# NVlabs/intrinsic3d

Measured on NVIDIA H100. Metric: gauss_newton_iterations_per_sec, higher is better.
Workload: dtype f32

## Files before the change

intrinsic3d_b200/csrc/i3d_engine.cu:

```cuda
#include <cuda_runtime.h>
#include <dlfcn.h>

#include <algorithm>
#include <chrono>
#include <climits>
#include <cmath>
#include <cstdarg>
#include <cstdio>
#include <cstdlib>
#include <cstring>
#include <string>
#include <vector>

#include "../../include/i3d_c_api.h"
#include "i3d_kernels.cuh"
#include "i3d_lighting.cuh"
#include "i3d_recolor.cuh"
#include "i3d_gridops.cuh"
#include "i3d_host.h"
#include "i3d_frames.h"
#include "i3d_fusion.h"
#include "i3d_mesh.h"
#include "i3d_render.h"
#include "i3d_texture.h"
#include "i3d_distance.h"
#include "i3d_grid_from_mesh.h"
#include "i3d_raster.h"
#include "i3d_track.h"

using namespace i3d;

#define I3D_ABI_VERSION 1

namespace
{
std::string g_create_error;

struct NcclApi
{
    typedef struct { char internal[128]; } UniqueId;
    typedef void* Comm;
    int (*GetUniqueId)(UniqueId*) = nullptr;
    int (*CommInitRank)(Comm*, int, UniqueId, int) = nullptr;
    int (*CommDestroy)(Comm) = nullptr;
    int (*AllReduce)(const void*, void*, size_t, int, int, Comm, cudaStream_t) = nullptr;
    const char* (*GetErrorString)(int) = nullptr;
    void* handle = nullptr;
    bool load(std::string* err)
    {
        if (handle) return true;
        const char* names[] = {"libnccl.so.2", "libnccl.so"};
        for (const char* nm : names) { handle = dlopen(nm, RTLD_NOW | RTLD_GLOBAL); if (handle) break; }
        if (!handle) { *err = std::string("cannot dlopen libnccl.so.2: ") + dlerror(); return false; }
        GetUniqueId = reinterpret_cast<decltype(GetUniqueId)>(dlsym(handle, "ncclGetUniqueId"));
        CommInitRank = reinterpret_cast<decltype(CommInitRank)>(dlsym(handle, "ncclCommInitRank"));
        CommDestroy = reinterpret_cast<decltype(CommDestroy)>(dlsym(handle, "ncclCommDestroy"));
        AllReduce = reinterpret_cast<decltype(AllReduce)>(dlsym(handle, "ncclAllReduce"));
        GetErrorString = reinterpret_cast<decltype(GetErrorString)>(dlsym(handle, "ncclGetErrorString"));
        if (!GetUniqueId || !CommInitRank || !CommDestroy || !AllReduce || !GetErrorString) { *err = "libnccl.so.2 lacks required symbols"; return false; }
        return true;
    }
};
NcclApi g_nccl;
// ... 287 lines not shown
    rows.n_active = e->n_active; rows.K = e->K; rows.stride = e->stride; rows.act = e->act.p; rows.Jt = e->Jt.p; rows.Jtail = e->Jtail.p;
    rows.row_frame = e->row_frame.p; rows.row_res = e->row_res.p; rows.row_wraw = e->row_wraw.p;
    return rows;
}

RegView reg_view(I3DEngine* e, const I3DParams& P)
{
    RegView rv;
    rv.flags = e->flags.p; rv.ea_w = e->ea_w.p; rv.lap = e->lap.p;
    rv.use_er = P.use_er; rv.use_es = P.use_es; rv.use_ea = P.use_ea;
    return rv;
}

SelectCam select_cam(const I3DEngine* e, const double hc9[9], float occlusion)
{
    SelectCam sc;
    sc.fx = static_cast<float>(hc9[0] * e->pyr_scale); sc.fy = static_cast<float>(hc9[1] * e->pyr_scale);
    sc.cx = static_cast<float>(hc9[2] * e->pyr_scale); sc.cy = static_cast<float>(hc9[3] * e->pyr_scale);
    sc.dist_zero = 1;
    for (int k = 0; k < 5; ++k) { sc.d[k] = static_cast<float>(hc9[4 + k]); if (sc.d[k] != 0.0f) sc.dist_zero = 0; }
    sc.occlusion = occlusion;
    return sc;
}

CullView cull_view(const I3DEngine* e, unsigned long long* stats)
{
    static const bool no_cull = std::getenv("I3D_NO_CULL") != nullptr;
    return CullView{e->tile_min.p, e->tile_max.p, no_cull ? 0 : 1, stats};
}

#define NK(call)                                                            \
    do {                                                                    \
        int _r = (call);                                                    \
        if (_r != 0) throw NcclError{_r, __LINE__};                         \
    } while (0)


bool pdl_enabled() { static const bool on = [] { const char* v = std::getenv("I3D_PDL"); return !(v && v[0] == '0'); }(); return on; }

template <bool COOPERATIVE = false, class... KArgs, class... Args>
void pdl_launch(I3DEngine* e, void (*kern)(KArgs...), unsigned grid, unsigned block, size_t smem, Args&&... args)
{
    cudaLaunchConfig_t cfg{};
    cfg.gridDim = dim3(grid); cfg.blockDim = dim3(block); cfg.dynamicSmemBytes = smem; cfg.stream = e->stream;
    cudaLaunchAttribute at[2];
    unsigned na = 0;
    if (COOPERATIVE) { at[na].id = cudaLaunchAttributeCooperative; at[na].val.cooperative = 1; ++na; }
    if (pdl_enabled()) { at[na].id = cudaLaunchAttributeProgrammaticStreamSerialization; at[na].val.programmaticStreamSerializationAllowed = 1; ++na; }
    cfg.attrs = at; cfg.numAttrs = na;
    CK(cudaLaunchKernelEx(&cfg, kern, static_cast<KArgs>(args)...));
    e->launches += 1;
}

template <int MODE>
void launch_eg_rows(I3DEngine* e, const GridView& g, const CamView& cv, const EgRows& rows, const int32_t* obs_frame, const float* obs_w)
{
    if constexpr (MODE == ROWS_COST)
    {
        const size_t smem = rows_smem_bytes(MODE, 256, true, e->F);
        if (2 * (smem + 1024) <= 227u * 1024u)
        {
            auto kern = k_eg_rows<MODE, 256, true>;
            CK(cudaFuncSetAttribute(kern, cudaFuncAttributeMaxDynamicSharedMemorySize, static_cast<int>(smem)));
            pdl_launch(e, kern, blocks_for(static_cast<size_t>(rows.stride), 256), 256, smem, g, e->frame_view(), cv, rows, obs_frame, obs_w, e->site(SITE_EG_COST));
            return;
        }
    }
    auto kern = k_eg_rows<MODE, 128, false>;
    const size_t smem = rows_smem_bytes(MODE, 128, false, e->F);
    CK(cudaFuncSetAttribute(kern, cudaFuncAttributeMaxDynamicSharedMemorySize, static_cast<int>(smem)));
    pdl_launch(e, kern, blocks_for(static_cast<size_t>(rows.stride), 128), 128, smem, g, e->frame_view(), cv, rows, obs_frame, obs_w, e->site(SITE_EG_COST));
}

void allreduce_scalars(I3DEngine* e, double* dev, int count, int kind, int respect_done)
{
    if (e->world <= 1) return;
    if (e->p2p_ready && count <= 30)
    {
        const unsigned int seq = ++e->xseq;
        pdl_launch(e, k_xchg_scalars, 1, 32, 0, e->p2p_view(), seq, dev, count, e->ctl.p, kind, respect_done);
        return;
    }
    NK(g_nccl.AllReduce(dev, dev, static_cast<size_t>(count), NCCL_FLOAT64, NCCL_SUM, e->comm, e->stream));
    if (kind >= 0) pdl_launch(e, k_epilogue, 1, 32, 0, e->ctl.p, dev, kind, respect_done);
}

void exchange(I3DEngine* e, float* v0, float* v1, float* extra_f, int n_extra_f, double* extra_d, int n_extra_d, int respect_done, int epilogue_kind = -1)
{
    if (e->world <= 1) return;
    const ShareView shv = e->share_view();
    const size_t nv = v1 ? 2 : 1;
    const size_t total = nv * static_cast<size_t>(e->n_shared) + n_extra_f + n_extra_d;
    const size_t threads = static_cast<size_t>(e->n_shared) + n_extra_f + n_extra_d;
    if (e->p2p_ready && total <= e->mbox_cap)
    {
        const unsigned int seq = ++e->xseq;
        double* buf = reinterpret_cast<double*>(e->mbox.p + I3DEngine::kMboxFlagBytes) + static_cast<size_t>(seq & 1u) * e->mbox_cap;
        pdl_launch(e, k_pack, blocks_for(threads), kThreads, 0, shv, v0, v1, extra_f, n_extra_f, extra_d, n_extra_d, buf, e->ctl.p, respect_done);
        pdl_launch(e, k_xchg_pull, blocks_for(threads), kThreads, 0, e->p2p_view(), seq, shv, v0, v1, extra_f, n_extra_f, extra_d, n_extra_d, e->ctl.p, respect_done, epilogue_kind);
        return;
    }
    e->xbuf.ensure(2 * static_cast<size_t>(e->n_shared) + CamAccLayout{e->F}.size() + 64);
    pdl_launch(e, k_pack, blocks_for(threads), kThreads, 0, shv, v0, v1, extra_f, n_extra_f, extra_d, n_extra_d, e->xbuf.p, e->ctl.p, respect_done);
    NK(g_nccl.AllReduce(e->xbuf.p, e->xbuf.p, total, NCCL_FLOAT64, NCCL_SUM, e->comm, e->stream));
    pdl_launch(e, k_unpack, blocks_for(threads), kThreads, 0, shv, v0, v1, extra_f, n_extra_f, extra_d, n_extra_d, e->xbuf.p, e->ctl.p, respect_done);
    if (epilogue_kind >= 0) pdl_launch(e, k_epilogue, 1, 32, 0, e->ctl.p, extra_d, epilogue_kind, respect_done);
// ... 70 lines not shown
        if (smem > dyn_max) break;
        int occ0 = 0, occ1 = 0;
        CK(cudaOccupancyMaxActiveBlocksPerMultiprocessor(&occ0, k_cg_step<false>, kStepThreads, smem));
        CK(cudaOccupancyMaxActiveBlocksPerMultiprocessor(&occ1, k_cg_step<true>, kStepThreads, smem));
        if (std::min(occ0, occ1) < bps) continue;
        if (static_cast<size_t>(bps) * sms + 8 > e->max_blocks) break;
        e->step_grid = static_cast<unsigned>(bps * sms); e->step_K = static_cast<int>(K); e->step_smem = smem;
        return true;
    }
    return false;
}

template <bool INIT>
void launch_cg_step(I3DEngine* e, const GridView& g, const RegView& rv, const SolveVecs& sv, float dmin, float dmax)
{
    const int64_t items = (e->n + 3) / 4;
    pdl_launch<true>(e, k_cg_step<INIT>, e->step_grid, kStepThreads, e->step_smem, g, rv, sv, items, e->step_K, e->type_w.p, e->minv.p, dmin, dmax,
                     e->ctl.p, e->site(SITE_OP_POST), e->site(SITE_EG_APPLY).out, e->site(SITE_UPDATE));
}

int gn_iteration_impl(I3DEngine* e, const I3DParams& P, I3DIterInfo& info)
{
    std::memset(&info, 0, sizeof(info));
    if (e->n <= 0) return fail(e, "i3d_gn_iteration: no grid uploaded");
    if (e->F <= 0) return fail(e, "i3d_gn_iteration: no frames uploaded");
    if (!e->have_cam) return fail(e, "i3d_gn_iteration: camera not set");
    if (!e->have_sh) return fail(e, "i3d_gn_iteration: SH coefficients not set");
    if (e->world > 1 && !e->shard_ready) return fail(e, "i3d_gn_iteration: world > 1 but i3d_set_shard was not called after the grid/frames upload");
    int K = P.num_observations;
    if (K <= 0 || K > e->F) K = e->F;
    if (K > I3D_MAX_OBS) return fail(e, "i3d_gn_iteration: num_observations (%d) exceeds I3D_MAX_OBS (%d)", K, I3D_MAX_OBS);
    if (P.lm_steps < 1) return fail(e, "i3d_gn_iteration: lm_steps < 1");
    if (P.residual_reset_period < 1) return fail(e, "i3d_gn_iteration: residual_reset_period < 1");
    if (check_frame_limit(e, e->F, K) != 0) return 1;
    e->K = K;
    e->last_params = P;
    e->timing.phases.clear(); begin_timing(e->timing, {}); e->launches = 0; e->host_syncs = 0;
    const int64_t n = e->n;
    const int F = e->F;
    const bool multi = e->world > 1;
    cudaStream_t st = e->stream;
    ensure_vectors(e);
    e->iter_dev.ensure(1);
    const Shard sh = e->shard();
    const int64_t own = sh.own_end - sh.own_begin;
    const int64_t hc = e->held_count();
    const size_t U = static_cast<size_t>(e->U());
    Timer t_total(e->timing, e->stream, "total");
    auto sync = [&]() { CK(cudaStreamSynchronize(st)); e->host_syncs += 1; };

    Timer t_sel(e->timing, e->stream, "select");
    e->flags.ensure(n);
    GridView g = e->grid_view(e->sdf, e->alb);
    pdl_launch(e, k_flags, blocks_for(static_cast<size_t>(sh.loc_end - sh.loc_begin)), kThreads, 0, g, sh, P.thres_shell, P.fix_all_albedo, e->flags.p);
    const int nscan = std::max(1, static_cast<int>((own + kScanChunk - 1) / kScanChunk));
    e->scan_counts.ensure(nscan); e->scan_total.ensure(1); e->act.ensure(n);
    pdl_launch(e, k_scan_count, nscan, kThreads, 0, own, e->flags.p + sh.own_begin, FL_ROW, e->scan_counts.p);
    pdl_launch(e, k_scan_blocks, 1, 1024, 0, nscan, e->scan_counts.p, e->scan_total.p);
    pdl_launch(e, k_scan_scatter, nscan, kThreads, 0, own, e->flags.p + sh.own_begin, FL_ROW, e->scan_counts.p, e->act.p, static_cast<int32_t>(sh.own_begin));
    const CamAccLayout lay{F};
    CK(cudaMemsetAsync(e->v_bg.p, 0, U * sizeof(float), st));
    CK(cudaMemsetAsync(e->v_cg.p, 0, U * sizeof(float), st));
    CK(cudaMemsetAsync(e->v_qg.p, 0, U * sizeof(float), st));
    CK(cudaMemsetAsync(e->v_delta.p, 0, U * sizeof(float), st));
    CK(cudaMemsetAsync(e->v_tr.p, 0, static_cast<size_t>(n) * sizeof(float), st));
    CK(cudaMemsetAsync(e->cam_acc.p, 0, lay.size() * sizeof(float), st));
    CK(cudaMemsetAsync(e->v_bgd.p, 0, U * sizeof(double), st));
    CK(cudaMemsetAsync(e->v_cgd.p, 0, U * sizeof(double), st));
    CK(cudaMemsetAsync(e->v_qgd.p, 0, U * sizeof(double), st));
    CK(cudaMemsetAsync(e->cam_accd.p, 0, lay.size() * sizeof(double), st));
    CK(cudaMemsetAsync(e->red_out.p, 0, 2 * kSiteVals * sizeof(double), st));
    e->Rt.ensure(12 * static_cast<size_t>(F));
    e->pose_ctx.ensure(F); e->pose_ctx_c.ensure(F);
    pdl_launch(e, k_pose_mats, blocks_for(F, 64), 64, 0, F, e->cam, e->Rt.p);
    pdl_launch(e, k_frame_pose, blocks_for(F, 64), 64, 0, F, e->cam, e->pose_ctx.p);
    int32_t n_active = 0;
    double hc9[9];
    CK(cudaMemcpyAsync(&n_active, e->scan_total.p, sizeof(int32_t), cudaMemcpyDeviceToHost, st));
    CK(cudaMemcpyAsync(hc9, e->cam + 6 * static_cast<size_t>(F), 9 * sizeof(double), cudaMemcpyDeviceToHost, st));
    sync();
    e->n_active = n_active;
    const int stride = (n_active + 63) & ~63;
    e->stride = stride;
    const size_t S = static_cast<size_t>(K) * stride;

    e->obs_frame.ensure(S + 1); e->obs_w.ensure(S + 1);
    if (n_active > 0)
    {
        const SelectCam sc = select_cam(e, hc9, P.occlusion_distance);
        const size_t smem = 12 * static_cast<size_t>(F) * sizeof(float);
        auto kern = (K <= 5) ? k_select_obs<5> : k_select_obs<I3D_MAX_OBS>;
        if (smem > 48 * 1024) CK(cudaFuncSetAttribute(kern, cudaFuncAttributeMaxDynamicSharedMemorySize, static_cast<int>(smem)));
        Timer kt(e->timing, e->stream, "k_select_obs");
        static const bool want_stats = std::getenv("I3D_CULL_STATS") != nullptr;
        e->cull_stats.ensure(2);
        if (want_stats) CK(cudaMemsetAsync(e->cull_stats.p, 0, 2 * sizeof(unsigned long long), st));
        const CullView cull = cull_view(e, want_stats ? e->cull_stats.p : nullptr);
        pdl_launch(e, kern, blocks_for(static_cast<size_t>(n_active)), kThreads, smem, g, e->frame_view(), e->Rt.p, sc, cull, n_active, stride, e->act.p, K,
                                                                                e->obs_frame.p, e->obs_w.p);
        if (want_stats)
        {
            unsigned long long hs[2] = {0, 0};
            CK(cudaMemcpyAsync(hs, e->cull_stats.p, sizeof(hs), cudaMemcpyDeviceToHost, st));
            CK(cudaStreamSynchronize(st));
            fprintf(stderr, "[i3d] frame culling: %llu of %llu (warp, frame) pairs visited (%.1f %%)\n", hs[0], hs[1], hs[1] ? 100.0 * hs[0] / hs[1] : 0.0);
        }
    }
    t_sel.stop();

    Timer t_build(e->timing, e->stream, "build");
    e->Jt.ensure(EgRows::kTiles * S + 1); e->Jtail.ensure(S + 1);
    e->row_frame.ensure(S + 1); e->row_res.ensure(S + 1); e->row_wraw.ensure(S + 1);
    e->ea_w.ensure(3 * static_cast<size_t>(n)); e->lap.ensure(n);
    CK(cudaFuncSetAttribute(k_eg_apply, cudaFuncAttributeMaxDynamicSharedMemorySize, static_cast<int>(apply_smem_bytes(F, K))));
    const EgRows rows = eg_rows(e);
    CamView cv{e->cam, e->pose_ctx.p, F};
    if (n_active > 0)
    {
        {
            Timer kt(e->timing, e->stream, "k_eg_build");
            launch_eg_rows<ROWS_BUILD>(e, g, cv, rows, e->obs_frame.p, e->obs_w.p);
        }
        const size_t smem = accum_smem_bytes(F, K);
        if (smem > 48 * 1024) CK(cudaFuncSetAttribute(k_eg_accum, cudaFuncAttributeMaxDynamicSharedMemorySize, static_cast<int>(smem)));
        {
            Timer kt(e->timing, e->stream, "k_eg_accum", 1);
            pdl_launch(e, k_eg_accum, blocks_for(static_cast<size_t>(n_active)), kThreads, smem, g, rows, F, e->v_bgd.p, e->v_cgd.p, e->cam_accd.p, e->site(SITE_BUILD));
        }
        pdl_launch(e, k_acc_to_float, blocks_for(std::max(U, static_cast<size_t>(lay.size()))), kThreads, 0, static_cast<int64_t>(U), lay.size(),
                   e->v_bgd.p, e->v_cgd.p, e->cam_accd.p, e->v_bg.p, e->v_cg.p, e->cam_acc.p);
    }
    const RegView rv = reg_view(e, P);
    pdl_launch(e, k_reg_build, blocks_for(static_cast<size_t>((sh.loc_end - sh.loc_begin + 3) / 4)), kThreads, 0, g, rv, sh, e->site(SITE_REG));
    {
        const double na = static_cast<double>(n_active);
        CK(cudaMemcpyAsync(e->site(SITE_BUILD).out + 3, &na, sizeof(double), cudaMemcpyHostToDevice, st));
    }
    if (multi) exchange(e, e->v_bg.p, e->v_cg.p, e->cam_acc.p, lay.size(), e->red_out.p, 2 * kSiteVals, 0);
    pdl_launch(e, k_type_weights, 1, 32, 0, e->iter_dev.p, e->site(SITE_BUILD).out, e->site(SITE_REG).out, P, n, e->type_w.p);
    if (S > 0) pdl_launch(e, k_row_weights, blocks_for(S), kThreads, 0, rows, e->type_w.p);
    SolveVecs sv = solve_vecs(e);
    pdl_launch(e, k_finish_problem, blocks_for(static_cast<size_t>((hc + 3) / 4)), kThreads, 0, g, rv, sv, sh, hc, e->type_w.p, e->cam_acc.p, P.fix_poses, P.fix_intrinsics,
                                                                              P.fix_distortion, P.gradient_tolerance, e->site(SITE_FINISH), e->cam);
    allreduce_scalars(e, e->site(SITE_FINISH).out, 3, -1, 0);
    pdl_launch(e, k_iter_finish, 1, 32, 0, e->iter_dev.p, e->site(SITE_FINISH).out, P);
    t_build.stop();
    e->have_iter = true;
    if (P.build_only)
    {
        IterDev hb{};
        CK(cudaMemcpyAsync(&hb, e->iter_dev.p, sizeof(hb), cudaMemcpyDeviceToHost, st));
        sync();
        CK(cudaGetLastError());
        info = hb.info;
        t_total.stop();
        return 0;
    }

    Timer t_solve(e->timing, e->stream, "solve");
    const float dmin = static_cast<float>(P.min_lm_diagonal), dmax = static_cast<float>(std::min(P.max_lm_diagonal, 3.0e38));
    const unsigned upd_blocks = blocks_for(static_cast<size_t>((sh.held_voxel_unknowns() + 3) / 4 + F + 2));
    auto launch_update = [&](bool init, int refresh) {
        if (init) pdl_launch(e, k_cg_update<true>, upd_blocks, kThreads, 0, sv, sh, e->minv.p, dmin, dmax, e->ctl.p, refresh, e->site(SITE_UPDATE));
        else pdl_launch(e, k_cg_update<false>, upd_blocks, kThreads, 0, sv, sh, e->minv.p, dmin, dmax, e->ctl.p, refresh, e->site(SITE_UPDATE));
    };
    const unsigned vec_blocks = blocks_for(static_cast<size_t>(hc));
    const int max_it = P.forced_cg_iterations > 0 ? P.forced_cg_iterations : P.max_linear_solver_iterations;
    const bool fused = e->pcg_fused && !multi && plan_cg_step(e);
    int enq = 0;
    bool dir_ready = false;
    auto enqueue_pcg = [&](int count) {
        for (int bidx = 0; bidx < count && enq < max_it; ++bidx)
        {
            ++enq;
            const bool refresh = (enq % P.residual_reset_period == 0);
            if (!dir_ready)
            {
                Timer kt(e->timing, e->stream, "k_cg_dir", 1);
                pdl_launch(e, k_cg_dir4, blocks_for(static_cast<size_t>((hc + 3) / 4)), kThreads, 0, sv, sh, hc, e->ctl.p);
            }
            dir_ready = false;
            if (fused && !refresh)
            {
                launch_eg_apply(e, g, rv, rows, sv);
                Timer kt(e->timing, e->stream, "k_cg_update", 1);
                launch_cg_step<false>(e, g, rv, sv, dmin, dmax);
                dir_ready = true;
                continue;
            }
            launch_operator(e, g, rv, rows, sv, sh, sv.p, dmin, dmax, 1);
            if (refresh)
            {
                pdl_launch(e, k_x_update, vec_blocks, kThreads, 0, sv, sh, hc, e->ctl.p);
                CK(cudaMemsetAsync(e->v_qg.p, 0, U * sizeof(float), st));
                pdl_launch(e, k_scale_vec, vec_blocks, kThreads, 0, sv, sh, hc, sv.x, 1.0f, sv.ps, e->ctl.p, 1);
                launch_operator(e, g, rv, rows, sv, sh, sv.x, dmin, dmax, 0);
                launch_update(false, 1);
            }
            else
            {
                Timer kt(e->timing, e->stream, "k_cg_update", 1);
                launch_update(false, 0);
            }
            if (multi) allreduce_scalars(e, e->site(SITE_UPDATE).out, 3, EPI_UPDATE, 1);
        }
    };
    auto enqueue_decision = [&]() {
        Timer t_cand(e->timing, e->stream, "candidate");
        CK(cudaMemsetAsync(e->red_out.p + SITE_CAND * kSiteVals, 0, 3 * kSiteVals * sizeof(double), st));
        pdl_launch(e, k_candidate, vec_blocks, kThreads, 0, g, sv, sh, hc, 0, e->cam, e->c_sdf, e->c_alb, e->c_cam, e->v_delta.p, e->ctl.p, e->site(SITE_CAND));
        GridView gc = e->grid_view(e->c_sdf, e->c_alb);
        pdl_launch(e, k_frame_pose, blocks_for(F, 64), 64, 0, F, e->c_cam, e->pose_ctx_c.p);
        CamView cvc{e->c_cam, e->pose_ctx_c.p, F};
        if (n_active > 0)
        {
            Timer kt(e->timing, e->stream, "k_eg_cost");
            launch_eg_rows<ROWS_COST>(e, gc, cvc, rows, nullptr, nullptr);
        }
        pdl_launch(e, k_reg_cost, blocks_for(static_cast<size_t>(own)), kThreads, 0, gc, rv, sh, e->c_sdf, e->c_alb, e->site(SITE_REG_COST));
        if (multi) allreduce_scalars(e, e->red_out.p + SITE_CAND * kSiteVals, 3 * kSiteVals, -1, 0);
        pdl_launch(e, k_lm_decide, 1, 32, 0, e->iter_dev.p, e->ctl.p, e->fail_flag.p, e->site(SITE_CAND).out, e->site(SITE_EG_COST).out,
                                      e->site(SITE_REG_COST).out, e->type_w.p, P);
    };
    IterDev h{};
    for (int it = 1; it <= P.lm_steps; ++it)
    {
        Timer t_pcg(e->timing, e->stream, "pcg");
        pdl_launch(e, k_lm_begin, 1, 32, 0, e->iter_dev.p, e->ctl.p, e->fail_flag.p, P);
        pdl_launch(e, k_cam_precond, blocks_for(static_cast<size_t>(F) + 2, 64), 64, 0, sv, e->cam_acc.p, e->type_w.p, e->ctl.p, dmin, dmax, e->minv.p, e->fail_flag.p);
        if (fused) launch_cg_step<true>(e, g, rv, sv, dmin, dmax);
        else launch_update(true, 0);
        dir_ready = fused;
        if (multi) allreduce_scalars(e, e->site(SITE_UPDATE).out, 3, EPI_UPDATE_INIT, 0);
        enq = 0;
        enqueue_pcg(P.forced_cg_iterations > 0 ? P.forced_cg_iterations : std::max(e->last_cg_iterations, e->prev_cg_iterations));
        t_pcg.stop();
        while (true)
        {
            enqueue_decision();
            CK(cudaMemcpyAsync(&h, e->iter_dev.p, sizeof(h), cudaMemcpyDeviceToHost, st));
            sync();
            CK(cudaGetLastError());
            if (!h.pcg_unfinished || h.state != LM_RUNNING) break;
            Timer t_more(e->timing, e->stream, "pcg");
            enqueue_pcg(2);
        }
        if (h.info.lm_iterations >= 1)
        {
            e->prev_cg_iterations = e->last_cg_iterations;
            e->last_cg_iterations = std::max(1, h.info.cg_iterations[std::min(h.info.lm_iterations - 1, I3D_MAX_LM_STEPS - 1)]);
        }
        if (h.state != LM_RUNNING) break;
    }
    info = h.info;
    if (h.precond_fail) e->error = "camera preconditioner block not SPD";
    if (h.state == LM_ACCEPTED)
    {
        if (multi)
        {
            pdl_launch(e, k_mask_owned, blocks_for(U), kThreads, 0, sv, sh, e->v_delta.p);
            NK(g_nccl.AllReduce(e->v_delta.p, e->v_delta.p, U, NCCL_FLOAT32, NCCL_SUM, e->comm, st));
            pdl_launch(e, k_candidate, blocks_for(U), kThreads, 0, g, sv, sh, static_cast<int64_t>(U), 1, e->cam, e->c_sdf, e->c_alb, e->c_cam, e->v_delta.p, e->ctl.p,
                                                           e->site(SITE_CAND));
            sync();
        }
        std::swap(e->sdf, e->c_sdf); std::swap(e->alb, e->c_alb); std::swap(e->cam, e->c_cam);
    }
    t_solve.stop();
    t_total.stop();
    return 0;
}

int setup_shard(I3DEngine* e)
{
    const int64_t n = e->n;
    const int64_t n2 = 2 * n;
    cudaStream_t st = e->stream;
    Shard sh0;
    sh0.own_begin = e->shard_begin; sh0.own_end = e->shard_end; sh0.hv0 = 0; sh0.hv1 = n; sh0.cam_owner = (e->rank == 0); sh0.defer = 1; sh0.loc_begin = 0; sh0.loc_end = n;
    Dev<uint8_t> touch, count;
    touch.ensure(n2); count.ensure(n2);
    CK(cudaMemsetAsync(touch.p, 0, n2, st));
// ... 2030 lines not shown
```

intrinsic3d_b200/csrc/i3d_kernels.cuh:

```cuda
#pragma once
#include <cuda_runtime.h>
#include <cooperative_groups.h>
#include <stdint.h>
#include <limits.h>
#include "i3d_math.cuh"
#include "i3d_grid.cuh"
#include "i3d_observe.cuh"
#include "../../include/i3d_types.h"

namespace i3d
{

enum : uint8_t { FL_VALID = 1, FL_ACTIVE = 2, FL_RING = 4, FL_FREE_SDF = 8, FL_FREE_ALB = 16, FL_ES_JAC = 32, FL_ROW = 64  };

struct Shard
{
    int64_t own_begin, own_end;
    int64_t hv0, hv1;
    int cam_owner;
    int defer;
    int64_t loc_begin, loc_end;
    __device__ __forceinline__ bool owns_voxel(int64_t v) const { return v >= own_begin && v < own_end; }
    __device__ __forceinline__ bool owns_unknown(int64_t j, int64_t n) const
    {
// ... 121 lines not shown
__device__ __forceinline__ int fk_select(const int (&fk)[I3D_MAX_OBS], int k)
{
    int r = fk[0];
#pragma unroll
    for (int i = 1; i < I3D_MAX_OBS; ++i) r = (k == i) ? fk[i] : r;
    return r;
}


__global__ void k_deinterleave_xyz(int64_t n, const int32_t* __restrict__ xyz, int32_t* __restrict__ x, int32_t* __restrict__ y, int32_t* __restrict__ z,
                                   const uint8_t* __restrict__ rgb3, uchar4* __restrict__ rgb4)
{
    const int64_t i = blockIdx.x * static_cast<int64_t>(blockDim.x) + threadIdx.x;
    if (i >= n) return;
    x[i] = xyz[3 * i]; y[i] = xyz[3 * i + 1]; z[i] = xyz[3 * i + 2];
    rgb4[i] = make_uchar4(rgb3[3 * i], rgb3[3 * i + 1], rgb3[3 * i + 2], 0);
}

__global__ void k_hash_insert(int64_t n, const int32_t* __restrict__ x, const int32_t* __restrict__ y, const int32_t* __restrict__ z,
                              unsigned long long* __restrict__ keys, int32_t* __restrict__ vals, uint64_t mask, int* __restrict__ dup_flag)
{
    const int64_t i = blockIdx.x * static_cast<int64_t>(blockDim.x) + threadIdx.x;
    if (i >= n) return;
    const unsigned long long key = pack_key(x[i], y[i], z[i]);
    uint64_t slot = mix64(key) & mask;
    while (true)
    {
        const unsigned long long prev = atomicCAS(&keys[slot], kEmptyKey, key);
        if (prev == kEmptyKey) { vals[slot] = static_cast<int32_t>(i); return; }
        if (prev == key) { atomicExch(dup_flag, 1); return; }
        slot = (slot + 1) & mask;
    }
}

__global__ void k_build_nbr(int64_t n, const int32_t* __restrict__ x, const int32_t* __restrict__ y, const int32_t* __restrict__ z,
                            const unsigned long long* __restrict__ keys, const int32_t* __restrict__ vals, uint64_t mask, int32_t* __restrict__ nbr)
{
    const int64_t i = blockIdx.x * static_cast<int64_t>(blockDim.x) + threadIdx.x;
    if (i >= n) return;
    const int X = x[i], Y = y[i], Z = z[i];
    const int off[NB_COUNT][3] = {{1, 0, 0}, {-1, 0, 0}, {0, 1, 0}, {0, -1, 0}, {0, 0, 1}, {0, 0, -1}, {2, 0, 0}, {0, 2, 0}, {0, 0, 2}, {1, 1, 0}, {1, 0, 1}, {0, 1, 1}};
#pragma unroll
    for (int o = 0; o < NB_COUNT; ++o) nbr[static_cast<int64_t>(o) * n + i] = hash_find(keys, vals, mask, X + off[o][0], Y + off[o][1], Z + off[o][2]);
}

__global__ void k_transpose_sh(int64_t n, const double* __restrict__ sh_aos, double* __restrict__ sh_soa)
{
    const int64_t i = blockIdx.x * static_cast<int64_t>(blockDim.x) + threadIdx.x;
    if (i >= 9 * n) return;
    const int64_t v = i / 9; const int k = static_cast<int>(i - 9 * v);
    sh_soa[static_cast<int64_t>(k) * n + v] = sh_aos[i];
}

__global__ void k_flags(GridView g, Shard sh, double thres_shell, int fix_all_albedo, uint8_t* __restrict__ flags)
{
    pdl_prologue();
    const int64_t v = sh.loc_begin + blockIdx.x * static_cast<int64_t>(blockDim.x) + threadIdx.x;
    if (v >= sh.loc_end) return;
    uint8_t fl = 0;
    const bool valid = g.weight[v] > 0.0f;
    if (valid) fl |= FL_VALID;
    bool ring = true;
#pragma unroll
    for (int o = 0; o < 6; ++o)
    {
        const int32_t nb = g.nbr[static_cast<int64_t>(o) * g.n + v];
        if (nb < 0 || !(g.weight[nb] > 0.0f)) ring = false;
    }
    if (ring) fl |= FL_RING;
    const double s = g.sdf[v];
    const bool inshell = !(fabs(s) > thres_shell);
    if (valid && inshell)
    {
        float nrm[3];
        if (surface_normal_f(g, v, nrm)) { fl |= FL_ACTIVE; if (sh.owns_voxel(v)) fl |= FL_ROW; }
        if (ring) { fl |= FL_FREE_SDF; if (!fix_all_albedo) fl |= FL_FREE_ALB; }
    }
    if ((s - g.sdf0[v]) != 0.0) fl |= FL_ES_JAC;
    flags[v] = fl;
}

constexpr int kScanItems = 8;
constexpr int kScanChunk = kThreads * kScanItems;

__global__ void k_scan_count(int64_t n, const uint8_t* __restrict__ flags, uint8_t bit, int32_t* __restrict__ block_counts)
{
    pdl_prologue();
    __shared__ int smem[32];
    const int64_t base = static_cast<int64_t>(blockIdx.x) * kScanChunk;
    int c = 0;
#pragma unroll
    for (int i = 0; i < kScanItems; ++i)
    {
        const int64_t idx = base + static_cast<int64_t>(i) * kThreads + threadIdx.x;
        if (idx < n && (flags[idx] & bit)) c++;
    }
    const int lane = threadIdx.x & 31, wid = threadIdx.x >> 5;
#pragma unroll
    for (int o = 16; o > 0; o >>= 1) c += __shfl_down_sync(0xffffffffu, c, o);
    if (lane == 0) smem[wid] = c;
    __syncthreads();
    if (threadIdx.x == 0)
    {
        int s = 0;
        for (int w = 0; w < kThreads / 32; ++w) s += smem[w];
        block_counts[blockIdx.x] = s;
    }
}

__global__ void k_scan_blocks(int nblocks, int32_t* __restrict__ block_counts, int32_t* __restrict__ total)
{
    pdl_prologue();
    __shared__ int carry;
    __shared__ int wsum[32];
    if (threadIdx.x == 0) carry = 0;
    __syncthreads();
    for (int base = 0; base < nblocks; base += blockDim.x)
    {
        const int i = base + threadIdx.x;
        const int v = (i < nblocks) ? block_counts[i] : 0;
        int incl = v;
        const int lane = threadIdx.x & 31, wid = threadIdx.x >> 5;
#pragma unroll
        for (int o = 1; o < 32; o <<= 1) { const int t = __shfl_up_sync(0xffffffffu, incl, o); if (lane >= o) incl += t; }
        if (lane == 31) wsum[wid] = incl;
        __syncthreads();
        if (wid == 0)
        {
            int w = (lane < (blockDim.x >> 5)) ? wsum[lane] : 0;
#pragma unroll
            for (int o = 1; o < 32; o <<= 1) { const int t = __shfl_up_sync(0xffffffffu, w, o); if (lane >= o) w += t; }
            wsum[lane] = w;
        }
        __syncthreads();
        const int woff = (wid > 0) ? wsum[wid - 1] : 0;
        const int excl = carry + woff + incl - v;
        if (i < nblocks) block_counts[i] = excl;
        __syncthreads();
        if (threadIdx.x == blockDim.x - 1) carry = excl + v;
        __syncthreads();
    }
    if (threadIdx.x == 0) *total = carry;
}

__global__ void k_scan_scatter(int64_t n, const uint8_t* __restrict__ flags, uint8_t bit, const int32_t* __restrict__ block_offsets,
                               int32_t* __restrict__ out_list, int32_t index_offset = 0)
{
    pdl_prologue();
    __shared__ int wsum[kThreads / 32];
    const int64_t base = static_cast<int64_t>(blockIdx.x) * kScanChunk;
    int running = block_offsets[blockIdx.x];
    const int lane = threadIdx.x & 31, wid = threadIdx.x >> 5;
    for (int i = 0; i < kScanItems; ++i)
    {
        const int64_t idx = base + static_cast<int64_t>(i) * kThreads + threadIdx.x;
        const bool f = idx < n && (flags[idx] & bit);
        const unsigned bal = __ballot_sync(0xffffffffu, f);
        if (lane == 0) wsum[wid] = __popc(bal);
        __syncthreads();
        int woff = 0, tot = 0;
        for (int w = 0; w < kThreads / 32; ++w) { const int c = wsum[w]; if (w < wid) woff += c; tot += c; }
        if (f) out_list[running + woff + __popc(bal & ((1u << lane) - 1u))] = static_cast<int32_t>(idx) + index_offset;
        running += tot;
        __syncthreads();
    }
}

__global__ void k_pose_mats(int F, const double* __restrict__ poses, float* __restrict__ Rt )
{
    pdl_prologue();
    const int f = blockIdx.x * blockDim.x + threadIdx.x;
    if (f >= F) return;
    const double wx = poses[6 * f], wy = poses[6 * f + 1], wz = poses[6 * f + 2];
    const double n2 = wx * wx + wy * wy + wz * wz;
    const double angle = sqrt(n2);
    double ax = wx, ay = wy, az = wz;
    if (n2 > 0.0) { ax = wx / angle; ay = wy / angle; az = wz / angle; }
    const double s = sin(angle), c = cos(angle);
    const double sx = __dmul_rn(s, ax), sy = __dmul_rn(s, ay), sz = __dmul_rn(s, az);
    const double c1x = __dmul_rn(1.0 - c, ax), c1y = __dmul_rn(1.0 - c, ay), c1z = __dmul_rn(1.0 - c, az);
    double M[9];
    double tmp;
    tmp = __dmul_rn(c1x, ay); M[1] = tmp - sz; M[3] = tmp + sz;
    tmp = __dmul_rn(c1x, az); M[2] = tmp + sy; M[6] = tmp - sy;
    tmp = __dmul_rn(c1y, az); M[5] = tmp - sx; M[7] = tmp + sx;
    M[0] = __dadd_rn(__dmul_rn(c1x, ax), c); M[4] = __dadd_rn(__dmul_rn(c1y, ay), c); M[8] = __dadd_rn(__dmul_rn(c1z, az), c);
    float* o = Rt + 12 * f;
#pragma unroll
    for (int i = 0; i < 9; ++i) o[i] = static_cast<float>(M[i]);
    o[9] = static_cast<float>(poses[6 * f + 3]); o[10] = static_cast<float>(poses[6 * f + 4]); o[11] = static_cast<float>(poses[6 * f + 5]);
}

__global__ void k_frame_pose(int F, const double* __restrict__ poses, FramePose* __restrict__ out)
{
    pdl_prologue();
// ... 527 lines not shown
                const bool act_b = fb & FL_ACTIVE, ring_b = fb & FL_RING;
                bool exists;
                if (active && act_b) exists = (v < b) ? ring : ring_b;
                else if (active) exists = ring;
                else if (act_b) exists = ring_b;
                else exists = false;
                if (exists && (fl & FL_VALID) && (fb & FL_VALID))
                {
                    float pw;
                    if (albedo_pair_weight(g.rgb[v], g.rgb[b], &pw) && pw != 0.0f)
                    {
                        w = pw;
                        const double r = g.albedo[v] - g.albedo[b];
                        if (own) { acc[4] += 1.0; acc[5] += static_cast<double>(pw); acc[6] += static_cast<double>(pw) * r * r; }
                    }
                }
            }
            rv.ea_w[static_cast<int64_t>(d) * g.n + v] = w;
        }
    }
    grid_reduce<9>(acc, site);
}

struct SolveVecs
{
    int64_t n; int F; int64_t U;
    float* bg;
    float* cg;
    float* s;
    float* jtj;
    float* b;
    float* x; float* r; float* z; float* p; float* ps; float* qg;
    double* qgd;
    float* tr;
};

struct TypeWeights { double w[4]; };

struct CgCtl
{
    double rho, last_rho, beta, alpha, pq, Q0, Q1, zeta;
    double xd2x;
    double inv_radius;
    int it;
    int done;
    int halt;
    int status;
    int forced_iterations, max_iterations, min_iterations;
    double eta;
    double model_cost_change, cand_cost, step_norm2, x_norm2;
};

__global__ void __launch_bounds__(kThreads)
k_finish_problem(GridView g, RegView rv, SolveVecs sv, Shard sh, int64_t count, const double* __restrict__ type_w, const float* __restrict__ cam_acc, int fix_poses,
                 int fix_intr, int fix_dist, double gradient_tolerance,
                 ReduceSite site ,
                 const double* __restrict__ cam)
{
    pdl_prologue();
    const int64_t tbase = (blockIdx.x * static_cast<int64_t>(blockDim.x) + threadIdx.x) * 4;
    double acc[3] = {0.0, 0.0, 0.0};
#pragma unroll
    for (int e4 = 0; e4 < 4; ++e4)
    {
        const int64_t t = tbase + e4;
        if (t >= count) break;
        const int64_t j = sh.unknown(t, sv.n);
        const double wg = type_w[0], wr = type_w[1], ws = type_w[2], wa = type_w[3];
        double c = 0.0, grad = 0.0, xval = 0.0;
        bool free_ = false;
        const int64_t n = g.n;
        if (j < n)
        {
            const int64_t v = j;
            const uint8_t fl = rv.flags[v];
            free_ = fl & FL_FREE_SDF;
            c = wg * static_cast<double>(sv.cg[j]); grad = wg * static_cast<double>(sv.bg[j]);
            const bool hasEr = rv.use_er && (fl & FL_ACTIVE) && (fl & FL_RING);
            if (rv.use_er)
            {
                double cnt = hasEr ? 36.0 : 0.0, gl = hasEr ? -6.0 * rv.lap[v] : 0.0;
#pragma unroll
                for (int o = 0; o < 6; ++o)
                {
                    const int32_t nb = g.nbr[static_cast<int64_t>(o) * n + v];
                    if (nb >= 0)
                    {
                        const uint8_t fb = rv.flags[nb];
                        if ((fb & FL_ACTIVE) && (fb & FL_RING)) { cnt += 1.0; gl += rv.lap[nb]; }
                    }
                }
                c += wr * cnt; grad += wr * gl;
            }
            if (rv.use_es && (fl & FL_ACTIVE) && (fl & FL_ES_JAC)) { c += ws; grad += ws * (g.sdf[v] - g.sdf0[v]); }
            xval = g.sdf[v];
        }
        else if (j < 2 * n)
        {
            const int64_t v = j - n;
            const uint8_t fl = rv.flags[v];
            free_ = fl & FL_FREE_ALB;
            c = wg * static_cast<double>(sv.cg[j]); grad = wg * static_cast<double>(sv.bg[j]);
            if (rv.use_ea)
            {
                const double av = g.albedo[v];
#pragma unroll
                for (int d = 0; d < 3; ++d)
                {
                    const float wp = rv.ea_w[static_cast<int64_t>(d) * n + v];
                    if (wp != 0.0f) { const int32_t b = g.nbr[static_cast<int64_t>(2 * d) * n + v]; c += wa * wp; grad += wa * wp * (av - g.albedo[b]); }
                    const int32_t m = g.nbr[static_cast<int64_t>(2 * d + 1) * n + v];
                    if (m >= 0)
                    {
                        const float wm = rv.ea_w[static_cast<int64_t>(d) * n + m];
                        if (wm != 0.0f) { c += wa * wm; grad += wa * wm * (av - g.albedo[m]); }
                    }
                }
            }
            xval = g.albedo[v];
        }
        else
        {
            const int64_t cidx = j - 2 * n;
            const CamAccLayout lay{sv.F};
            if (cidx < 6 * static_cast<int64_t>(sv.F))
            {
                const int f = static_cast<int>(cidx / 6), k = static_cast<int>(cidx - 6 * f);
                free_ = !fix_poses;
                grad = wg * static_cast<double>(cam_acc[lay.pose_stride() * f + k]);
                c = wg * static_cast<double>(cam_acc[lay.pose_stride() * f + 6 + k]);
            }
            else
            {
                const int k = static_cast<int>(cidx - 6 * static_cast<int64_t>(sv.F));
                free_ = (k < 4) ? !fix_intr : !fix_dist;
                grad = wg * static_cast<double>(cam_acc[lay.tail() + k]);
                c = wg * static_cast<double>(cam_acc[lay.tail() + 9 + k]);
            }
            xval = cam[cidx];
        }
        const double s = free_ ? 1.0 / (1.0 + sqrt(c)) : 0.0;
        sv.s[j] = static_cast<float>(s);
        sv.jtj[j] = static_cast<float>(s * s * c);
        sv.b[j] = static_cast<float>(s * grad);
        if (sh.owns_unknown(j, n))
        {
            if (free_ && c > 0.0) { acc[0] += 1.0; acc[1] += xval * xval; }
            if (free_ && fabs(grad) > gradient_tolerance) acc[2] += 1.0;
        }
    }
    grid_reduce<3>(acc, site);
}

__device__ __forceinline__ float lm_diag(float jtj, float dmin, float dmax) { return fminf(fmaxf(jtj, dmin), dmax); }

struct CamBlock { int m; int64_t base; size_t moff; };
__device__ __forceinline__ CamBlock cam_block(int blk, int F, int64_t n)
{
    const int64_t c0 = 2 * n + 6 * static_cast<int64_t>(F);
    if (blk < F) return {6, 2 * n + 6 * static_cast<int64_t>(blk), 36 * static_cast<size_t>(blk)};
    if (blk == F) return {4, c0, 36 * static_cast<size_t>(F)};
    return {5, c0 + 4, 36 * static_cast<size_t>(F) + 16};
}

__device__ inline bool chol_inverse(int m, double* A , double* inv)
{
    for (int i = 0; i < m; ++i)
        for (int j = 0; j <= i; ++j)
        {
            double s = A[i * m + j];
            for (int k = 0; k < j; ++k) s -= A[i * m + k] * A[j * m + k];
            if (i == j) { if (!(s > 0.0)) return false; A[i * m + i] = sqrt(s); }
            else A[i * m + j] = s / A[j * m + j];
        }
    for (int c = 0; c < m; ++c)
    {
        double y[6], x[6];
        for (int i = 0; i < m; ++i)
        {
            double s = (i == c) ? 1.0 : 0.0;
            for (int k = 0; k < i; ++k) s -= A[i * m + k] * y[k];
            y[i] = s / A[i * m + i];
        }
        for (int i = m - 1; i >= 0; --i)
        {
            double s = y[i];
            for (int k = i + 1; k < m; ++k) s -= A[k * m + i] * x[k];
            x[i] = s / A[i * m + i];
        }
        for (int i = 0; i < m; ++i) inv[i * m + c] = x[i];
// ... 1154 lines not shown
```

Measured before the change: 140.9.

## Fold accumulator clears and double-to-float conversion into existing build kernels

On a single device, the zeroing of the double accumulators moves into k_flags, the active count is written as a double by k_scan_blocks, and the k_acc_to_float pass is folded into k_finish_problem, which reads the double sums directly. Several memsets, an H2D copy and a conversion kernel are dropped from the single-GPU path, and each launch gets per-kernel timing wrappers. This trades launch and memset overhead for extra stores in k_flags and conditional reads in k_finish_problem. Correctness depends on the cleared buffers and the float cam_acc copy not being needed elsewhere before they are rewritten.

Result: no change. 140.9, median of 6 (-0.0%).

```diff
diff --git a/intrinsic3d_b200/csrc/i3d_engine.cu b/intrinsic3d_b200/csrc/i3d_engine.cu
--- a/intrinsic3d_b200/csrc/i3d_engine.cu
+++ b/intrinsic3d_b200/csrc/i3d_engine.cu
@@ -9,6 +9,7 @@
 #include <cstdio>
 #include <cstdlib>
 #include <cstring>
+#include <utility>
 #include <string>
 #include <vector>
 
@@ -402,6 +403,13 @@
     e->launches += 1;
 }
 
+template <bool COOPERATIVE = false, class... KArgs, class... Args>
+void pdl_launch_named(I3DEngine* e, const char* name, void (*kern)(KArgs...), unsigned grid, unsigned block, size_t smem, Args&&... args)
+{
+    Timer kt(e->timing, e->stream, name, 1);
+    pdl_launch<COOPERATIVE>(e, kern, grid, block, smem, std::forward<Args>(args)...);
+}
+
 template <int MODE>
 void launch_eg_rows(I3DEngine* e, const GridView& g, const CamView& cv, const EgRows& rows, const int32_t* obs_frame, const float* obs_w)
 {
@@ -578,34 +586,45 @@
     Timer t_sel(e->timing, e->stream, "select");
     e->flags.ensure(n);
     GridView g = e->grid_view(e->sdf, e->alb);
-    pdl_launch(e, k_flags, blocks_for(static_cast<size_t>(sh.loc_end - sh.loc_begin)), kThreads, 0, g, sh, P.thres_shell, P.fix_all_albedo, e->flags.p);
+    const CamAccLayout lay{F};
+    const EgAccum acc{e->v_bgd.p, e->v_cgd.p, e->cam_accd.p, lay.size()};
+    const EgAccum no_acc{nullptr, nullptr, nullptr, 0};
+    pdl_launch_named(e, "k_flags", k_flags, blocks_for(static_cast<size_t>(sh.loc_end - sh.loc_begin)), kThreads, 0, g, sh, P.thres_shell, P.fix_all_albedo, e->flags.p,
+                     multi ? no_acc : acc);
     const int nscan = std::max(1, static_cast<int>((own + kScanChunk - 1) / kScanChunk));
     e->scan_counts.ensure(nscan); e->scan_total.ensure(1); e->act.ensure(n);
-    pdl_launch(e, k_scan_count, nscan, kThreads, 0, own, e->flags.p + sh.own_begin, FL_ROW, e->scan_counts.p);
-    pdl_launch(e, k_scan_blocks, 1, 1024, 0, nscan, e->scan_counts.p, e->scan_total.p);
-    pdl_launch(e, k_scan_scatter, nscan, kThreads, 0, own, e->flags.p + sh.own_begin, FL_ROW, e->scan_counts.p, e->act.p, static_cast<int32_t>(sh.own_begin));
-    const CamAccLayout lay{F};
-    CK(cudaMemsetAsync(e->v_bg.p, 0, U * sizeof(float), st));
-    CK(cudaMemsetAsync(e->v_cg.p, 0, U * sizeof(float), st));
+    pdl_launch_named(e, "k_scan_count", k_scan_count, nscan, kThreads, 0, own, e->flags.p + sh.own_begin, FL_ROW, e->scan_counts.p);
+    pdl_launch_named(e, "k_scan_blocks", k_scan_blocks, 1, 1024, 0, nscan, e->scan_counts.p, e->scan_total.p, multi ? nullptr : e->site(SITE_BUILD).out + 3);
+    pdl_launch_named(e, "k_scan_scatter", k_scan_scatter, nscan, kThreads, 0, own, e->flags.p + sh.own_begin, FL_ROW, e->scan_counts.p, e->act.p, static_cast<int32_t>(sh.own_begin));
+    Timer t_clear(e->timing, e->stream, "memset_select", 1);
+    if (multi)
+    {
+        CK(cudaMemsetAsync(e->v_bg.p, 0, U * sizeof(float), st));
+        CK(cudaMemsetAsync(e->v_cg.p, 0, U * sizeof(float), st));
+        CK(cudaMemsetAsync(e->cam_acc.p, 0, lay.size() * sizeof(float), st));
+        CK(cudaMemsetAsync(e->v_bgd.p, 0, U * sizeof(double), st));
+        CK(cudaMemsetAsync(e->v_cgd.p, 0, U * sizeof(double), st));
+        CK(cudaMemsetAsync(e->cam_accd.p, 0, lay.size() * sizeof(double), st));
+        CK(cudaMemsetAsync(e->red_out.p, 0, 2 * kSiteVals * sizeof(double), st));
+    }
+    if (multi || P.build_only) CK(cudaMemsetAsync(e->v_delta.p, 0, U * sizeof(float), st));
     CK(cudaMemsetAsync(e->v_qg.p, 0, U * sizeof(float), st));
-    CK(cudaMemsetAsync(e->v_delta.p, 0, U * sizeof(float), st));
     CK(cudaMemsetAsync(e->v_tr.p, 0, static_cast<size_t>(n) * sizeof(float), st));
-    CK(cudaMemsetAsync(e->cam_acc.p, 0, lay.size() * sizeof(float), st));
-    CK(cudaMemsetAsync(e->v_bgd.p, 0, U * sizeof(double), st));
-    CK(cudaMemsetAsync(e->v_cgd.p, 0, U * sizeof(double), st));
     CK(cudaMemsetAsync(e->v_qgd.p, 0, U * sizeof(double), st));
-    CK(cudaMemsetAsync(e->cam_accd.p, 0, lay.size() * sizeof(double), st));
-    CK(cudaMemsetAsync(e->red_out.p, 0, 2 * kSiteVals * sizeof(double), st));
+    t_clear.stop();
     e->Rt.ensure(12 * static_cast<size_t>(F));
     e->pose_ctx.ensure(F); e->pose_ctx_c.ensure(F);
-    pdl_launch(e, k_pose_mats, blocks_for(F, 64), 64, 0, F, e->cam, e->Rt.p);
-    pdl_launch(e, k_frame_pose, blocks_for(F, 64), 64, 0, F, e->cam, e->pose_ctx.p);
+    pdl_launch_named(e, "k_pose_mats", k_pose_mats, blocks_for(F, 64), 64, 0, F, e->cam, e->Rt.p);
+    pdl_launch_named(e, "k_frame_pose", k_frame_pose, blocks_for(F, 64), 64, 0, F, e->cam, e->pose_ctx.p);
     int32_t n_active = 0;
     double hc9[9];
+    Timer t_drain(e->timing, e->stream, "drain_select", 1);
     CK(cudaMemcpyAsync(&n_active, e->scan_total.p, sizeof(int32_t), cudaMemcpyDeviceToHost, st));
     CK(cudaMemcpyAsync(hc9, e->cam + 6 * static_cast<size_t>(F), 9 * sizeof(double), cudaMemcpyDeviceToHost, st));
     sync();
+    t_drain.stop();
     e->n_active = n_active;
+    if (!multi && n_active == 0) CK(cudaMemsetAsync(e->site(SITE_BUILD).out, 0, 3 * sizeof(double), st));
     const int stride = (n_active + 63) & ~63;
     e->stride = stride;
     const size_t S = static_cast<size_t>(K) * stride;
@@ -653,23 +672,26 @@
             Timer kt(e->timing, e->stream, "k_eg_accum", 1);
             pdl_launch(e, k_eg_accum, blocks_for(static_cast<size_t>(n_active)), kThreads, smem, g, rows, F, e->v_bgd.p, e->v_cgd.p, e->cam_accd.p, e->site(SITE_BUILD));
         }
-        pdl_launch(e, k_acc_to_float, blocks_for(std::max(U, static_cast<size_t>(lay.size()))), kThreads, 0, static_cast<int64_t>(U), lay.size(),
+        if (multi) pdl_launch_named(e, "k_acc_to_float", k_acc_to_float, blocks_for(std::max(U, static_cast<size_t>(lay.size()))), kThreads, 0, static_cast<int64_t>(U), lay.size(),
                    e->v_bgd.p, e->v_cgd.p, e->cam_accd.p, e->v_bg.p, e->v_cg.p, e->cam_acc.p);
     }
     const RegView rv = reg_view(e, P);
-    pdl_launch(e, k_reg_build, blocks_for(static_cast<size_t>((sh.loc_end - sh.loc_begin + 3) / 4)), kThreads, 0, g, rv, sh, e->site(SITE_REG));
+    pdl_launch_named(e, "k_reg_build", k_reg_build, blocks_for(static_cast<size_t>((sh.loc_end - sh.loc_begin + 3) / 4)), kThreads, 0, g, rv, sh, e->site(SITE_REG));
+    if (multi)
     {
         const double na = static_cast<double>(n_active);
+        Timer kt(e->timing, e->stream, "h2d_na", 1);
         CK(cudaMemcpyAsync(e->site(SITE_BUILD).out + 3, &na, sizeof(double), cudaMemcpyHostToDevice, st));
     }
     if (multi) exchange(e, e->v_bg.p, e->v_cg.p, e->cam_acc.p, lay.size(), e->red_out.p, 2 * kSiteVals, 0);
-    pdl_launch(e, k_type_weights, 1, 32, 0, e->iter_dev.p, e->site(SITE_BUILD).out, e->site(SITE_REG).out, P, n, e->type_w.p);
-    if (S > 0) pdl_launch(e, k_row_weights, blocks_for(S), kThreads, 0, rows, e->type_w.p);
+    pdl_launch_named(e, "k_type_weights", k_type_weights, 1, 32, 0, e->iter_dev.p, e->site(SITE_BUILD).out, e->site(SITE_REG).out, P, n, e->type_w.p);
+    if (S > 0) pdl_launch_named(e, "k_row_weights", k_row_weights, blocks_for(S), kThreads, 0, rows, e->type_w.p);
     SolveVecs sv = solve_vecs(e);
-    pdl_launch(e, k_finish_problem, blocks_for(static_cast<size_t>((hc + 3) / 4)), kThreads, 0, g, rv, sv, sh, hc, e->type_w.p, e->cam_acc.p, P.fix_poses, P.fix_intrinsics,
-                                                                              P.fix_distortion, P.gradient_tolerance, e->site(SITE_FINISH), e->cam);
+    pdl_launch_named(e, "k_finish_problem", k_finish_problem, blocks_for(std::max(static_cast<size_t>((hc + 3) / 4), static_cast<size_t>(lay.size()))), kThreads, 0,
+                     g, rv, sv, sh, hc, e->type_w.p, e->cam_acc.p, multi ? no_acc : acc, P.fix_poses, P.fix_intrinsics, P.fix_distortion, P.gradient_tolerance,
+                     e->site(SITE_FINISH), e->cam);
     allreduce_scalars(e, e->site(SITE_FINISH).out, 3, -1, 0);
-    pdl_launch(e, k_iter_finish, 1, 32, 0, e->iter_dev.p, e->site(SITE_FINISH).out, P);
+    pdl_launch_named(e, "k_iter_finish", k_iter_finish, 1, 32, 0, e->iter_dev.p, e->site(SITE_FINISH).out, P);
     t_build.stop();
     e->have_iter = true;
     if (P.build_only)
@@ -733,27 +755,31 @@
     };
     auto enqueue_decision = [&]() {
         Timer t_cand(e->timing, e->stream, "candidate");
-        CK(cudaMemsetAsync(e->red_out.p + SITE_CAND * kSiteVals, 0, 3 * kSiteVals * sizeof(double), st));
-        pdl_launch(e, k_candidate, vec_blocks, kThreads, 0, g, sv, sh, hc, 0, e->cam, e->c_sdf, e->c_alb, e->c_cam, e->v_delta.p, e->ctl.p, e->site(SITE_CAND));
+        if (multi || n_active == 0)
+        {
+            Timer kt(e->timing, e->stream, "memset_cand", 1);
+            CK(cudaMemsetAsync(e->red_out.p + SITE_CAND * kSiteVals, 0, 3 * kSiteVals * sizeof(double), st));
+        }
+        pdl_launch_named(e, "k_candidate", k_candidate, vec_blocks, kThreads, 0, g, sv, sh, hc, 0, e->cam, e->c_sdf, e->c_alb, e->c_cam, e->v_delta.p, e->ctl.p, e->site(SITE_CAND));
         GridView gc = e->grid_view(e->c_sdf, e->c_alb);
-        pdl_launch(e, k_frame_pose, blocks_for(F, 64), 64, 0, F, e->c_cam, e->pose_ctx_c.p);
+        pdl_launch_named(e, "k_frame_pose_cand", k_frame_pose, blocks_for(F, 64), 64, 0, F, e->c_cam, e->pose_ctx_c.p);
         CamView cvc{e->c_cam, e->pose_ctx_c.p, F};
         if (n_active > 0)
         {
             Timer kt(e->timing, e->stream, "k_eg_cost");
             launch_eg_rows<ROWS_COST>(e, gc, cvc, rows, nullptr, nullptr);
         }
-        pdl_launch(e, k_reg_cost, blocks_for(static_cast<size_t>(own)), kThreads, 0, gc, rv, sh, e->c_sdf, e->c_alb, e->site(SITE_REG_COST));
+        pdl_launch_named(e, "k_reg_cost", k_reg_cost, blocks_for(static_cast<size_t>(own)), kThreads, 0, gc, rv, sh, e->c_sdf, e->c_alb, e->site(SITE_REG_COST));
         if (multi) allreduce_scalars(e, e->red_out.p + SITE_CAND * kSiteVals, 3 * kSiteVals, -1, 0);
-        pdl_launch(e, k_lm_decide, 1, 32, 0, e->iter_dev.p, e->ctl.p, e->fail_flag.p, e->site(SITE_CAND).out, e->site(SITE_EG_COST).out,
+        pdl_launch_named(e, "k_lm_decide", k_lm_decide, 1, 32, 0, e->iter_dev.p, e->ctl.p, e->fail_flag.p, e->site(SITE_CAND).out, e->site(SITE_EG_COST).out,
                                       e->site(SITE_REG_COST).out, e->type_w.p, P);
     };
     IterDev h{};
     for (int it = 1; it <= P.lm_steps; ++it)
     {
         Timer t_pcg(e->timing, e->stream, "pcg");
-        pdl_launch(e, k_lm_begin, 1, 32, 0, e->iter_dev.p, e->ctl.p, e->fail_flag.p, P);
-        pdl_launch(e, k_cam_precond, blocks_for(static_cast<size_t>(F) + 2, 64), 64, 0, sv, e->cam_acc.p, e->type_w.p, e->ctl.p, dmin, dmax, e->minv.p, e->fail_flag.p);
+        pdl_launch_named(e, "k_lm_begin", k_lm_begin, 1, 32, 0, e->iter_dev.p, e->ctl.p, e->fail_flag.p, P);
+        pdl_launch_named(e, "k_cam_precond", k_cam_precond, blocks_for(static_cast<size_t>(F) + 2, 64), 64, 0, sv, e->cam_acc.p, e->type_w.p, e->ctl.p, dmin, dmax, e->minv.p, e->fail_flag.p);
         if (fused) launch_cg_step<true>(e, g, rv, sv, dmin, dmax);
         else launch_update(true, 0);
         dir_ready = fused;
diff --git a/intrinsic3d_b200/csrc/i3d_kernels.cuh b/intrinsic3d_b200/csrc/i3d_kernels.cuh
--- a/intrinsic3d_b200/csrc/i3d_kernels.cuh
+++ b/intrinsic3d_b200/csrc/i3d_kernels.cuh
@@ -197,11 +197,18 @@
     sh_soa[static_cast<int64_t>(k) * n + v] = sh_aos[i];
 }
 
-__global__ void k_flags(GridView g, Shard sh, double thres_shell, int fix_all_albedo, uint8_t* __restrict__ flags)
+struct EgAccum { double* bg; double* cg; double* cam; int ncam; };
+
+__global__ void k_flags(GridView g, Shard sh, double thres_shell, int fix_all_albedo, uint8_t* __restrict__ flags, EgAccum clear)
 {
     pdl_prologue();
     const int64_t v = sh.loc_begin + blockIdx.x * static_cast<int64_t>(blockDim.x) + threadIdx.x;
     if (v >= sh.loc_end) return;
+    if (clear.bg)
+    {
+        clear.bg[v] = 0.0; clear.bg[g.n + v] = 0.0; clear.cg[v] = 0.0; clear.cg[g.n + v] = 0.0;
+        for (int64_t i = v; i < clear.ncam; i += g.n) clear.cam[i] = 0.0;
+    }
     uint8_t fl = 0;
     const bool valid = g.weight[v] > 0.0f;
     if (valid) fl |= FL_VALID;
@@ -253,7 +260,7 @@
     }
 }
 
-__global__ void k_scan_blocks(int nblocks, int32_t* __restrict__ block_counts, int32_t* __restrict__ total)
+__global__ void k_scan_blocks(int nblocks, int32_t* __restrict__ block_counts, int32_t* __restrict__ total, double* __restrict__ total_d = nullptr)
 {
     pdl_prologue();
     __shared__ int carry;
@@ -285,7 +292,7 @@
         if (threadIdx.x == blockDim.x - 1) carry = excl + v;
         __syncthreads();
     }
-    if (threadIdx.x == 0) *total = carry;
+    if (threadIdx.x == 0) { *total = carry; if (total_d) *total_d = static_cast<double>(carry); }
 }
 
 __global__ void k_scan_scatter(int64_t n, const uint8_t* __restrict__ flags, uint8_t bit, const int32_t* __restrict__ block_offsets,
@@ -919,13 +926,17 @@
 };
 
 __global__ void __launch_bounds__(kThreads)
-k_finish_problem(GridView g, RegView rv, SolveVecs sv, Shard sh, int64_t count, const double* __restrict__ type_w, const float* __restrict__ cam_acc, int fix_poses,
-                 int fix_intr, int fix_dist, double gradient_tolerance,
+k_finish_problem(GridView g, RegView rv, SolveVecs sv, Shard sh, int64_t count, const double* __restrict__ type_w, float* __restrict__ cam_acc, EgAccum eg,
+                 int fix_poses, int fix_intr, int fix_dist, double gradient_tolerance,
                  ReduceSite site ,
                  const double* __restrict__ cam)
 {
     pdl_prologue();
-    const int64_t tbase = (blockIdx.x * static_cast<int64_t>(blockDim.x) + threadIdx.x) * 4;
+    const int64_t tid = blockIdx.x * static_cast<int64_t>(blockDim.x) + threadIdx.x;
+    const int64_t tbase = tid * 4;
+    const bool from_double = eg.bg != nullptr;
+    if (from_double && tid < eg.ncam) cam_acc[tid] = static_cast<float>(eg.cam[tid]);
+    auto cam_sum = [&](int i) { return from_double ? static_cast<float>(eg.cam[i]) : cam_acc[i]; };
     double acc[3] = {0.0, 0.0, 0.0};
 #pragma unroll
     for (int e4 = 0; e4 < 4; ++e4)
@@ -942,7 +953,8 @@
             const int64_t v = j;
             const uint8_t fl = rv.flags[v];
             free_ = fl & FL_FREE_SDF;
-            c = wg * static_cast<double>(sv.cg[j]); grad = wg * static_cast<double>(sv.bg[j]);
+            const float cgj = from_double ? static_cast<float>(eg.cg[j]) : sv.cg[j], bgj = from_double ? static_cast<float>(eg.bg[j]) : sv.bg[j];
+            c = wg * static_cast<double>(cgj); grad = wg * static_cast<double>(bgj);
             const bool hasEr = rv.use_er && (fl & FL_ACTIVE) && (fl & FL_RING);
             if (rv.use_er)
             {
@@ -967,7 +979,8 @@
             const int64_t v = j - n;
             const uint8_t fl = rv.flags[v];
             free_ = fl & FL_FREE_ALB;
-            c = wg * static_cast<double>(sv.cg[j]); grad = wg * static_cast<double>(sv.bg[j]);
+            const float cgj = from_double ? static_cast<float>(eg.cg[j]) : sv.cg[j], bgj = from_double ? static_cast<float>(eg.bg[j]) : sv.bg[j];
+            c = wg * static_cast<double>(cgj); grad = wg * static_cast<double>(bgj);
             if (rv.use_ea)
             {
                 const double av = g.albedo[v];
@@ -994,15 +1007,15 @@
             {
                 const int f = static_cast<int>(cidx / 6), k = static_cast<int>(cidx - 6 * f);
                 free_ = !fix_poses;
-                grad = wg * static_cast<double>(cam_acc[lay.pose_stride() * f + k]);
-                c = wg * static_cast<double>(cam_acc[lay.pose_stride() * f + 6 + k]);
+                grad = wg * static_cast<double>(cam_sum(lay.pose_stride() * f + k));
+                c = wg * static_cast<double>(cam_sum(lay.pose_stride() * f + 6 + k));
             }
             else
             {
                 const int k = static_cast<int>(cidx - 6 * static_cast<int64_t>(sv.F));
                 free_ = (k < 4) ? !fix_intr : !fix_dist;
-                grad = wg * static_cast<double>(cam_acc[lay.tail() + k]);
-                c = wg * static_cast<double>(cam_acc[lay.tail() + 9 + k]);
+                grad = wg * static_cast<double>(cam_sum(lay.tail() + k));
+                c = wg * static_cast<double>(cam_sum(lay.tail() + 9 + k));
             }
             xval = cam[cidx];
         }
```
